# NeLy-EPFL/flygym

Measured on AMD Instinct MI355X. Metric: env-steps/sec (whole node), 4096 flies per GPU, flat terrain, higher is better.
Workload: dtype f32

## Files before the change

flygym_amd/csrc/nmf_capi.hip:

```cpp
#include <algorithm>
#include <cmath>
#include <cstdio>
#include <cstdlib>
#include <cstring>
#include <string>
#include <vector>

#ifndef NMF_DEVMEM_CHECK
#include <hip/hip_runtime.h>

#include "nmf.h"
#include "nmf_batch_ops.hip"
#include "nmf_step.hip"
#include "nmf_sensors.hip"
#include "nmf_eyes.hip"
#include "nmf_camera.hip"
#include "nmf_replay.hip"
#include "nmf_cpg.hip"
#include "nmf_skeleton.h"
#endif

namespace {

thread_local std::string g_err;
// ... 330 lines not shown
      std::vector<int> trn = model->find("act_trn")->i;
      for (int u = 0; u < model->nu; ++u) if ((int)ag->f[(size_t)u * nmf::kActGen] & 1) trn[(size_t)u] = 0;
      upload(b, trn, &d.act_trn);
    }
  }
  UI(geom_body); UI(geom_type); UI(geom_hulladr); UI(geom_hullnum); UI(geom_sensor);
  UF(geom_p0); UF(geom_p1); UF(geom_radius); UF(geom_bsphere); UF(geom_invweight0); UF(hull_vert);
  UF(pair_friction); UF(pair_solref); UF(pair_solimp); UF(pair_margin);
#undef UF
#undef UI
  if (fam.tree_tables()) {
    const HostArray* bp = model->find("body_parent");
    upload(b, bp->i, &d.body_parent);
    upload(b, tree_body, &d.tree_body);
    upload(b, child_start, &d.tree_child_start);
    upload(b, child_count, &d.tree_child_count);
    d.tree_nlevel = (int)lvl_start.size() - 1;
    for (size_t k = 0; k < 18; ++k) d.tree_lvl_start[k] = k < lvl_start.size() ? lvl_start[k] : (int)tree_body.size();
    d.rest_fast = 0; d.rest_pack = nullptr;
    std::vector<int> pack;
    if (fam.hybrid() && !opt.rest_slow && rest_pack_words(model, sk, pack)) { d.rest_fast = 1; upload(b, pack, &d.rest_pack); }
  } else {
    d.body_parent = d.tree_body = d.tree_child_start = d.tree_child_count = nullptr; d.tree_nlevel = 0; d.rest_fast = 0; d.rest_pack = nullptr;
  }
  d.noslip_iter = 0;
  if (const HostArray* os2 = model->find("opt_solver")) { if (os2->i.size() > 1) d.noslip_iter = os2->i[1]; }
  d.max_contacts = nmf::kMaxCon;
  d.solver_flags = opt.solver & 7;
  if (rc != 0) return rc;
  b->dm_dev = (nmf::DevModel*)b->mem.upload(&d, sizeof(nmf::DevModel));
  return b->mem.ok ? 0 : -1;
}

int alloc_state(nmf_batch* b) {
  const nmf_model* model = b->model;
  const size_t n_worlds = (size_t)b->n_worlds;
  nmf::DevState& st = b->st;
  st.n_worlds = b->n_worlds;
  float* stats_sum = nullptr;
  b->handoff_stride = (model->nq + 2 * model->nv + model->nu + 6 + nmf::kActHistWords + 63) / 64 * 64;
  alloc_field(b, NMF_QPOS, model->nq, &st.qpos); alloc_field(b, NMF_QVEL, model->nv, &st.qvel);
  alloc_field(b, NMF_CTRL, model->nu, &st.ctrl); alloc_field(b, NMF_QACC_WARMSTART, model->nv, &st.qacc_ws);
  alloc_field(b, NMF_SEG_XPOS, model->nseg * 3, &st.seg_xpos); alloc_field(b, NMF_SEG_XQUAT, model->nseg * 4, &st.seg_xquat);
  alloc_field(b, NMF_SITE_XPOS, model->nsite * 3, &st.site_xpos); alloc_field(b, NMF_ACTUATOR_FORCE, model->nu, &st.actuator_force);
  alloc_field(b, NMF_SENSORDATA, 96, &st.sensordata); alloc_field(b, NMF_TIME, 1, &st.time);
  alloc_field(b, NMF_STATS, 8, &st.stats); alloc_field(b, NMF_QACC, model->nv, &st.qacc); alloc_field(b, NMF_COST, 1, &st.cost);
  alloc_field(b, NMF_STATS_SUM, 16, &stats_sum);
  alloc_field(b, NMF_CONTACT_GEOM, nmf::kMaxCon, &st.contact_geom); alloc_field(b, NMF_ACT, model->nu, &st.act);
  alloc_dev(b, n_worlds, &b->order_buf); alloc_dev(b, 1, &b->csched_buf);
  alloc_dev(b, n_worlds * (size_t)b->handoff_stride, &b->handoff_buf);
  alloc_dev(b, n_worlds * nmf::kActHistWords, &st.act_hist);
  st.stats_sum = reinterpret_cast<unsigned int*>(stats_sum);
  st.dual_scratch = nullptr;
  with_topo(b->topo, [&](auto tag) { if (nmf::kDualGlob<typename decltype(tag)::type>) alloc_dev(b, n_worlds * nmf::kDualScratchFloats, &st.dual_scratch); });
  st.noslip_buf = nullptr;
  if (b->dm.noslip_iter > 0) alloc_dev(b, n_worlds * nmf::kNoslipFloats, &st.noslip_buf);
  alloc_dev(b, 2, &b->clock_probe_buf); alloc_dev(b, 1, &b->sched_buf);
  st.clock_probe = b->clock_probe_buf;
  st.sched = nullptr;
  st.order = nullptr;
  return b->mem.ok ? 0 : -1;
}

void set_schedule(nmf_batch* b, const Options& opt) {
  b->chunking = opt.sched != 1;
  if (opt.order) b->order_policy = opt.order == 1 ? 0 : opt.order == 2 ? 1 : opt.order == 3 ? 2 : opt.order == 4 ? -1 : 3;
  if (opt.order_every > 0) b->order_every = opt.order_every;
  if (opt.max_chunks > 0) b->max_chunks = std::max(1, std::min(16, opt.max_chunks));
  b->chunk_div = b->dm.terrain_type == 0 ? nmf::family(b->topo).chunk_div : 2.0;
  b->chunk_div_short = true;
  if (opt.chunk_div > 0.0) { b->chunk_div = opt.chunk_div; b->chunk_div_short = false; }
  if (opt.min_chunk_steps > 0) b->min_chunk_steps = opt.min_chunk_steps;
  if (b->dm.act_general) b->chunking = false;
}

int pick_kernel(nmf_batch* b, const Options& opt) {
  const int topo = b->topo, device = b->mem.device;
  int per_cu = nmf::family(topo).per_cu;
  const bool weld = b->dm.weld_active != 0, terrain = b->dm.terrain_type != 0;
  if (weld && terrain) return fail("nmf_batch_create: a tethered world has no terrain");
  const void* fn = step_kernel(topo, weld, terrain);
  if (!fn) return fail("nmf_batch_create: this build of the library has no kernel for the model's skeleton (NMF_TOPO_MASK)");
  int nblk = 0;
  if (hipOccupancyMaxActiveBlocksPerMultiprocessor(&nblk, fn, nmf::kWave, 0) == hipSuccess && nblk > 0) per_cu = nblk;
  b->step_fn = fn;
  const int want = opt.flies_per_cu;
  hipFuncAttributes fa;
  if (want > 0 && want < per_cu && hipFuncGetAttributes(&fa, fn) == hipSuccess) {
    int lds_cu = 0;
    if (hipDeviceGetAttribute(&lds_cu, hipDeviceAttributeMaxSharedMemoryPerMultiprocessor, device) != hipSuccess || lds_cu <= 0) lds_cu = 160 * 1024;
    const int granule = 512;
    int per_wg = (lds_cu / (want + 1) / granule + 1) * granule;
    if (per_wg * want <= lds_cu && per_wg > (int)fa.sharedSizeBytes) {
      b->lds_pad = (unsigned)(per_wg - (int)fa.sharedSizeBytes);
      int nblk2 = 0;
      if (hipOccupancyMaxActiveBlocksPerMultiprocessor(&nblk2, fn, nmf::kWave, b->lds_pad) == hipSuccess && nblk2 > 0) per_cu = std::min(per_cu, nblk2);
      else per_cu = want;
    }
  }
  if (const char* e = dev_env("NMF_LDS_PAD")) b->lds_pad = (unsigned)atoi(e);
  b->per_cu = per_cu;
  hipDeviceProp_t prop;
  b->resident_waves = (hipGetDeviceProperties(&prop, device) == hipSuccess ? prop.multiProcessorCount : 256) * per_cu;
  return 0;
}

}
// ... 807 lines not shown
```

flygym_amd/csrc/nmf_step.hip:

```cpp
#include "nmf_device.h"
#include "nmf_step_lds.h"
#include "nmf_step_diag.h"
#include "nmf_step_kinematics.h"
#include "nmf_step_collision.h"
#include "nmf_step_aba.h"
#include "nmf_step_contact.h"
#include "nmf_dual.h"
#include "nmf_step_noslip.h"
#include "nmf_step_actuation.h"
#include "nmf_step_forward.h"
#include "nmf_step_io.h"
#include "nmf_tree.h"

namespace nmf {

template <class TP> constexpr int waves_per_simd() { return 2; }

template <class TP>
__device__ __forceinline__ void stage_launch_constants(FlyLds<TP>& s, const GModel& m) {
  if constexpr (!TP::kStar) { if (threadIdx.x == 0) { s.rt_nb = m.nb; s.rt_nv = m.nv; } __syncthreads(); }
  if constexpr (TP::kNFact > 1) {
    for (int b = threadIdx.x; b < TP::kTblB && b < m.nb; b += kWave) {
      s.t_body[b] = (unsigned char)m.tree_body[b < m.tree_lvl_start[m.tree_nlevel] ? b : 0];
      s.t_parent[b] = (unsigned char)(b ? m.body_parent[b] : 0);
// ... 31 lines not shown
      }
    }
  }
  if constexpr (kHasIsym<TP>) if (lane == 0) {
    const Frame fr = make_frame(v3(m.plane[0], m.plane[1], m.plane[2]));
    st3(&s.frame9[0], fr.n); st3(&s.frame9[3], fr.t1); st3(&s.frame9[6], fr.t2);
    HotModel& h = s.hot;
    h.dof_axis = m.dof_axis; h.body_pos = m.body_pos; h.body_quat = m.body_quat; h.geom_p0 = m.geom_p0; h.geom_p1 = m.geom_p1;
    h.geom_radius = m.geom_radius; h.geom_bsphere = m.geom_bsphere; h.hull_vert = m.hull_vert; h.pair_margin = m.pair_margin;
    h.geom_body = m.geom_body; h.geom_type = m.geom_type; h.geom_hulladr = m.geom_hulladr; h.geom_hullnum = m.geom_hullnum;
#pragma unroll
    for (int i = 0; i < 4; ++i) h.plane[i] = m.plane[i];
#pragma unroll
    for (int i = 0; i < 5; ++i) h.terrain[i] = m.terrain[i];
    h.hull_skin = m.hull_skin; h.terrain_type = m.terrain_type; h.ng = m.ng; h.sem_max_hull_contacts = m.sem_max_hull_contacts;
    h.terrain_walls = m.sem_terrain_walls;
  }
  if constexpr (kHasIsym<TP>) for (int i = lane; i < 3 * s.nv(); i += kWave) (&s.axis[0][0])[i] = m.dof_axis[i];
}

template <class TP>
__global__ void __launch_bounds__(kWave) nmf_reset_kernel(const DevModel* __restrict__ mp, DevState st, const unsigned char* __restrict__ reset_mask) {
  __shared__ FlyLds<TP> s;
  const GModel& m = *(const GModel*)mp;
  const int lane = threadIdx.x, w = (int)blockIdx.x;
  if (w >= st.n_worlds || (reset_mask && !reset_mask[w])) return;
  stage_launch_constants(s, m);
  for (int i = lane; i < s.nq(); i += kWave) s.qpos[i] = m.key_qpos[i];
  for (int i = lane; i < s.nv(); i += kWave) { s.qvel[i] = 0.f; s.qacc[i] = 0.f; }
  for (int i = lane; i < m.nu; i += kWave) { s.ctrl[i] = m.key_ctrl[i]; st.actuator_force[(size_t)w * m.nu + i] = 0.f; st.act[(size_t)w * m.nu + i] = 0.f; }
  for (int i = lane; i < 96; i += kWave) st.sensordata[(size_t)w * 96 + i] = 0.f;
  if (lane == 0) { s.ncon = 0; s.iters = 0; s.overflow = 0; s.solve_resid = 0.f; }
  WSYNC();
  stage_kinematics(s, m, lane);
  write_poses(s, m, st, w, lane);
  write_outputs(s, m, st, w, lane, 0.f, true);
  if (lane < 16) st.stats_sum[16 * (size_t)w + lane] = 0u;
  if (lane < kActHistWords) st.act_hist[(size_t)w * kActHistWords + lane] = 0u;
  if (lane < kMaxCon) st.contact_geom[(size_t)w * kMaxCon + lane] = -1.f;
}

template <class TP, bool WELD>
__global__ void __launch_bounds__(kWave) __attribute__((amdgpu_waves_per_eu(waves_per_simd<TP>(), waves_per_simd<TP>()))) nmf_step_kernel(const DevModel* __restrict__ mp, DevState st, ReplayArgs rp, int n_steps) {
  __shared__ FlyLds<TP> s;
  const GModel& m = *(const GModel*)mp;
  const unsigned long long probe_c0 = __builtin_amdgcn_s_memtime(), probe_r0 = __builtin_amdgcn_s_memrealtime();
  TRACE_DECL();
  const int lane = threadIdx.x;
  const bool chunked = st.sched_mode == 1;
  unsigned int t_first = 0;
  if (chunked && lane == 0) t_first = atomicAdd(&st.csched->ticket, 1u);
  stage_launch_constants(s, m);
  if constexpr (kDualGlob<TP>) { if (lane == 0) s.dual_glob[0] = st.dual_scratch + (size_t)blockIdx.x * kDualScratchFloats; }
  unsigned int t_next = (unsigned int)__builtin_amdgcn_readfirstlane((int)t_first);
  STAGE_INIT();
  const int n_chunks = chunked ? st.n_chunks : 1;
  const unsigned int epoch = chunked ? (unsigned int)__builtin_amdgcn_readfirstlane((int)st.csched->epoch) : 0u;
  for (;;) {
    int slot = (int)blockIdx.x, chunk = 0, step0 = 0, step1 = n_steps;
    if (chunked) {
      const unsigned int t = t_next;
      if (t >= (unsigned int)st.n_worlds * (unsigned int)n_chunks) {
        if (lane == 0 && atomicAdd(&st.csched->exited, 1u) == gridDim.x - 1u) {
          st.csched->ticket = 0u; st.csched->exited = 0u; st.csched->epoch = epoch + 1u;
        }
        break;
      }
      chunk = (int)(t / (unsigned int)st.n_worlds); slot = (int)(t % (unsigned int)st.n_worlds);
      step0 = st.chunk_start[chunk]; step1 = st.chunk_start[chunk + 1];
    } else if (slot >= st.n_worlds) return;
    const int w = __builtin_amdgcn_readfirstlane(st.order ? st.order[slot] : slot);
    TRACE_SUB(2);
    const unsigned long long t_begin = __builtin_amdgcn_s_memtime();
    if (st.sched && lane == 0) atomicMin(&st.sched->t_first, (unsigned long long)__builtin_amdgcn_s_memrealtime());
    float time;
    unsigned int carry = 0u;
    unsigned int sum_con = 0u, sum_it = 0u, sum_of = 0u;
    unsigned int sum_dual = 0u, sum_kkt = 0u;
    {
      const float* tab = rp.table ? rp.table + (size_t)w * rp.table_steps * rp.n_act : nullptr;
      const int ln = opaque(lane);
      const int my_ctrl = tab && lane < rp.n_act ? rp.act_ids[ln] : -1;
      CtrlPrefetch pf;
      pf.mine = my_ctrl >= 0; pf.next_row = nullptr;
      pf.value = my_ctrl >= 0 ? tab[(size_t)((rp.start + step0) % rp.table_steps) * rp.n_act + lane] : 0.f;
      if (chunk > 0) {
        const unsigned int want = (unsigned int)__builtin_amdgcn_readfirstlane((int)(epoch * 32u + (unsigned int)chunk));
        const unsigned long long* hb = st.handoff + (size_t)w * st.handoff_stride;
        const int nq = s.nq(), nv = s.nv();
        for (;;) {
          bool ok = true;
          for (int i = ln; i < nq; i += kWave) s.qpos[i] = ld_tagged(&hb[i], want, ok);
          for (int i = ln; i < nv; i += kWave) { s.qvel[i] = ld_tagged(&hb[nq + i], want, ok); s.qacc[i] = ld_tagged(&hb[nq + nv + i], want, ok); }
          for (int i = ln; i < m.nu; i += kWave) s.ctrl[i] = ld_tagged(&hb[nq + 2 * nv + i], want, ok);
          carry = lane < 6 ? ld_tagged_u(&hb[nq + 2 * nv + m.nu + ln], want, ok) : 0u;
          if constexpr (kDual<TP>) { const unsigned int hw = lane < hist_words<TP>(m) ? ld_tagged_u(&hb[nq + 2 * nv + m.nu + 6 + ln], want, ok) : 0u; if (lane < kHistLds<TP>) s.act_hist[lane] = hw; }
          if (!__any(!ok)) break;
          __builtin_amdgcn_s_sleep(8);
        }
        time = __uint_as_float((unsigned int)__builtin_amdgcn_readlane((int)carry, 0));
      } else {
        for (int i = ln; i < s.nq(); i += kWave) s.qpos[i] = ld_state(&st.qpos[(size_t)w * s.nq() + i]);
        for (int i = ln; i < s.nv(); i += kWave) {
          s.qvel[i] = ld_state(&st.qvel[(size_t)w * s.nv() + i]);
          s.qacc[i] = ld_state(&st.qacc_ws[(size_t)w * s.nv() + i]);
        }
// ... 77 lines not shown
```

flygym_amd/csrc/nmf_step_aba.h:

```cpp
#pragma once
#include "nmf_device.h"

namespace nmf {

template <class TP> __device__ void tree_sweep_twists(FlyLds<TP>& s, const float* x, float (*T)[row_width_tw<TP>()], const GModel& m, int lane);
template <class TP, class Extra, class Emit>
__device__ __forceinline__ void tree_sweep_project(FlyLds<TP>& s, float (*W)[row_width_tw<TP>()], const GModel& m, int lane, Extra&& extra, Emit&& emit);
template <class TP, bool WELD>
__device__ void tree_aba_solve(FlyLds<TP>& s, int tau_id, int x_id, bool withK, float hdamp, const GModel& m, int lane);
template <class TP> __device__ void tree_sweep_twists_levels(FlyLds<TP>& s, const float* x, float (*T)[row_width_tw<TP>()], const GModel& m, int lane);
template <class TP, class Extra>
__device__ __forceinline__ void tree_gather_levels(FlyLds<TP>& s, float (*W)[row_width_tw<TP>()], const GModel& m, int lane, Extra&& extra);
struct RestNode;
template <class TP, bool FAST, bool UP, class F> __device__ __forceinline__ void rest_levels(FlyLds<TP>& s, int lane, F&& f);
template <class TP, int NUM>
__device__ __forceinline__ void rest_aba_eliminate(FlyLds<TP>& s, const RestNode& nd, const float* tau, bool withK, float hdamp,
                                                   const Frame& fr, const LaneRole& L, const int (&so)[6], const struct InertiaRowMap& IM, const GModel& m);
template <class TP, int NUM, bool HOMOGENEOUS>
__device__ __forceinline__ void rest_aba_expand(FlyLds<TP>& s, const RestNode& nd, float* x, const LaneRole& L);

template <class TP>
__device__ __forceinline__ bool rest_reduced(const FlyLds<TP>& s) {
  if constexpr (TP::kStar) { if constexpr (TP::REST_B > 0) return __builtin_amdgcn_readfirstlane(s.reduced) != 0; }
  return false;
// ... 231 lines not shown
  const float invD = __builtin_amdgcn_rcpf(D);
  const float u = tauj - sp;
  const float k = U * invD;
  const f2 nk = mk2(-k, -k);
  a01 = __builtin_elementwise_fma(nk, mk2(grp8_bcast<0>(U), grp8_bcast<1>(U)), a01);
  a23 = __builtin_elementwise_fma(nk, mk2(grp8_bcast<2>(U), grp8_bcast<3>(U)), a23);
  a45 = __builtin_elementwise_fma(nk, mk2(grp8_bcast<4>(U), grp8_bcast<5>(U)), a45);
  IA[0] = a01.x; IA[1] = a01.y; IA[2] = a23.x; IA[3] = a23.y; IA[4] = a45.x; IA[5] = a45.y;
  pA += k * u;
  UDout = SHADOW0 ? k : mask * k; uDout = u * invD;
  Uraw = U; invDraw = invD;
}
typedef const __attribute__((address_space(3))) float* lds_cptr;
template <class T>
__device__ __forceinline__ lds_cptr lds_pinned(const T* p) {
  lds_cptr q = (lds_cptr)(const void*)p;
  asm("" : "+v"(q));
  return q;
}

template <class TP> __device__ __forceinline__ float (*dual_leg(FlyLds<TP>& s))[8] {
  if constexpr (kDualGlob<TP>) return reinterpret_cast<float(*)[8]>(s.dual_glob[0]);
  else if constexpr (kDualH<TP>) {
    static_assert(!kDualH<TP> || kDualGlob<TP> || 4 * TP::NV >= TP::NLEG * TP::NDL * 8, "leg factors do not fit vA..vD");
    return reinterpret_cast<float(*)[8]>(&s.vA[0]);
  } else {
    static_assert(sizeof(float) * 8 * (TP::NLEG * TP::NDL + 6) <= sizeof(float) * 12 * kMaxCon, "articulated-body factors do not fit c_w + c_m3");
    return reinterpret_cast<float(*)[8]>(&s.c_w[0][0]);
  }
}
template <class TP> __device__ __forceinline__ float (*dual_root(FlyLds<TP>& s))[8] {
  if constexpr (kDualH<TP>) return reinterpret_cast<float(*)[8]>(&s.c_w[0][0]);
  else return dual_leg(s) + TP::NLEG * TP::NDL;
}
template <class TP> __device__ __forceinline__ float* dual_aref(FlyLds<TP>& s) {
  if constexpr (kDualH<TP>) return &s.c_w[0][0] + 48; else return s.vB;
}
template <class TP> __device__ __forceinline__ float (*dual_wrench(FlyLds<TP>& s))[7] {
  if constexpr (kDualH<TP>) {
    static_assert(!kDualH<TP> || 7 * kDualMaxCon<TP> <= TP::NV, "contact wrenches do not fit vC");
    return reinterpret_cast<float(*)[7]>(&s.vC[0]);
  } else return s.c_w;
}
template <class TP> __device__ __forceinline__ float* dual_acc(FlyLds<TP>& s) {
  if constexpr (kDualH<TP>) {
    static_assert(!kDualH<TP> || 96 + TP::NLEG * TP::NDL + 6 <= 7 * kMaxCon, "hinge sums do not fit c_w");
    return &s.c_w[0][0] + 96;
  } else {
    static_assert(TP::NLEG * TP::NDL + 6 <= 3 * TP::NV, "hinge sums do not fit vB..vD");
    return s.vB;
  }
}

template <class TP, bool WELD, bool WITHK_ = true>
__device__ __noinline__ void aba_solve(FlyLds<TP>& s, int tau_id, int x_id, bool withK, float hdamp,
                          const GModel& m, int lane, bool store = false, bool withF = false) {
  if constexpr (!TP::kStar) { tree_aba_solve<TP, WELD>(s, tau_id, x_id, withK, hdamp, m, lane); return; } else {
  withK = WITHK_ && __builtin_amdgcn_readfirstlane((int)withK) != 0;
  store = kDual<TP> && __builtin_amdgcn_readfirstlane((int)store) != 0;
  withF = kDual<TP> && __builtin_amdgcn_readfirstlane((int)withF) != 0;
  const float* tau = s.vec(tau_id);
  float* x = s.vec(x_id);
  Frame fr{};
  if (withK) fr = ld_frame(s, m);
  const bool walls = TP::kTerrain && withK && __builtin_amdgcn_readfirstlane(s.nwall) != 0;
  const LaneRole L = lane_role<TP>(lane);
  const int j0 = TP::LD0 + L.lg * TP::NDL, b0 = TP::LB0 + L.lg * TP::NBL;
  static_assert(sizeof(AbaHandoff<TP>) <= sizeof(float) * TP::NB * 12, "ABA hand-off does not fit T..W");
  AbaHandoff<TP>& H = *reinterpret_cast<AbaHandoff<TP>*>(&s.T[0][0]);
  int so[6];
#pragma unroll
  for (int c = 0; c < 6; c++) {
    if constexpr (kHasIsym<TP>) so[c] = __float_as_int(s.k_tab[L.rr][14 + c]);
    else { const int i = L.rr < c ? L.rr : c, jx = L.rr < c ? c : L.rr; so[c] = i * 6 - i * (i - 1) / 2 + (jx - i); }
  }
  InertiaRowMap IM{};
  if constexpr (!kHasIsym<TP>) IM = inertia_map_unpack(s.k_tab[L.rr]);
  constexpr bool kKeepS = TP::NDL <= 16;
  float Ureg[TP::NDL], ureg[TP::NDL], Sreg[kKeepS ? TP::NDL : 1];
  constexpr bool kShadow0 = row_width_s<TP>() > 6 && row_width_tw<TP>() > 6;
  const int rS = kShadow0 && L.r >= 6 ? 6 : L.rr;
  const lds_cptr Sleg = lds_pinned(&s.S[j0][0]), Sown = lds_pinned(&s.S[j0][rS]);
  constexpr int SW = row_width_s<TP>();
  KLane KL;
  if (withK) {
    const float* q = s.k_tab[L.rr];
#pragma unroll
    for (int i = 0; i < 3; ++i) { KL.dA[i] = q[i]; KL.dB[i] = q[3 + i]; KL.dO[i] = q[6 + i]; }
    KL.ia = __float_as_int(q[9]); KL.ib = __float_as_int(q[10]);
  }
  int cs[TP::NBL + 1], cs_root0 = 0, cs_root1 = 0;
  static_for<TP::NBL + 1>([&](auto I) { constexpr int l = decltype(I)::value; cs[l] = withK || withF ? s.body_cstart[b0 + l] : 0; });
  if (withK || withF) { cs_root0 = s.body_cstart[0]; cs_root1 = s.body_cstart[1]; }
  const bool red = rest_reduced(s);
  SUB_T0();
  if constexpr (TP::REST_B > 0) {
    if (!red) {
      if (m.rest_fast) rest_levels<TP, true, true>(s, lane, [&](const auto& nd) { rest_aba_eliminate<TP, 3>(s, nd, tau, withK, hdamp, fr, L, so, IM, m); });
      else rest_levels<TP, false, true>(s, lane, [&](const auto& nd) { rest_aba_eliminate<TP, 0>(s, nd, tau, withK, hdamp, fr, L, so, IM, m); });
      WSYNC();
    }
  }
  SUB(18);
  float IA[6] = {0.f, 0.f, 0.f, 0.f, 0.f, 0.f};
  float pA = 0.f;
  float n_sj[6], n_sown = 0.f, n_delta = 0.f, n_tau = 0.f, n_row[6];
  auto fetch_hinge = [&](auto DN) {
    constexpr int dn = decltype(DN)::value;
#pragma unroll
    for (int i = 0; i < 6; i++) n_sj[i] = Sleg[dn * SW + i];
    n_sown = Sown[dn * SW];
    n_delta = dof_delta(s, m, j0 + dn, hdamp);
    n_tau = tau[j0 + dn];
    if constexpr (TP::is_last(dn) && kHasIsym<TP>) {
#pragma unroll
      for (int c = 0; c < 6; c++) n_row[c] = s.Isym[b0 + TP::lbody(dn)][so[c]];
    }
  };
  fetch_hinge(std::integral_constant<int, TP::NDL - 1>{});
  static_for<TP::NDL>([&](auto DD) {
    constexpr int d = TP::NDL - 1 - decltype(DD)::value;
    float sj[6], row[6];
#pragma unroll
    for (int i = 0; i < 6; i++) { sj[i] = n_sj[i]; row[i] = n_row[i]; }
    const float sown = n_sown, delta = n_delta, tj = n_tau;
    if constexpr (d > 0) fetch_hinge(std::integral_constant<int, (d > 0 ? d - 1 : 0)>{});
    if constexpr (TP::is_last(d)) {
      const int b = b0 + TP::lbody(d);
      if constexpr (kHasIsym<TP>) {
        if constexpr (kDual<TP>) {
          if (withF) {
#pragma clang loop unroll(disable) vectorize(disable)
            for (int c = cs[TP::lbody(d)]; c < cs[TP::lbody(d) + 1]; ++c) pA -= dual_wrench(s)[c][L.rr];
          }
        }
        if (withK) for (int c = cs[TP::lbody(d)]; c < cs[TP::lbody(d) + 1]; ++c) add_contact_K_row(row, s, c, KL, fr, L.rr, walls);
        add6(IA, row);
      } else {
        add_inertia_row(IA, s, b, IM);
        if constexpr (kDual<TP>) {
          if (withF) {
#pragma clang loop unroll(disable) vectorize(disable)
            for (int c = cs[TP::lbody(d)]; c < cs[TP::lbody(d) + 1]; ++c) pA -= dual_wrench(s)[c][L.rr];
          }
        }
        if (withK) for (int c = cs[TP::lbody(d)]; c < cs[TP::lbody(d) + 1]; ++c) add_contact_K_row(IA, s, c, KL, fr, L.rr, walls);
      }
    }
    const float sr = kShadow0 ? sown : L.mask * sown;
    if constexpr (kKeepS) Sreg[d] = sown;
    float Uraw, invDraw;
    aba_step_scaled<kShadow0>(IA, pA, sj, sr, L.mask, delta, tj, Ureg[d], ureg[d], Uraw, invDraw);
    if constexpr (kDual<TP>) {
      if (store) {
        const float rs = __builtin_sqrtf(invDraw);
        if constexpr (kDualGlob<TP>) ((__attribute__((address_space(1))) float*)s.dual_glob[0])[(L.lg * TP::NDL + d) * 8 + (L.r < 6 ? L.r : 6)] = L.r < 6 ? Uraw * rs : rs;
        else dual_leg(s)[L.lg * TP::NDL + d][L.r < 6 ? L.r : 6] = L.r < 6 ? Uraw * rs : rs;
      }
    }
  });
  constexpr bool kLegSumValu = TP::NLEG <= 8;
  float legs_row[6] = {0.f, 0.f, 0.f, 0.f, 0.f, 0.f}, legs_pA = 0.f;
  if constexpr (kLegSumValu) {
    const float gm = L.grp < TP::NLEG ? 1.f : 0.f;
#pragma unroll
    for (int i = 0; i < 6; i++) legs_row[i] = groups_sum(gm * IA[i]);
    legs_pA = groups_sum(gm * pA);
  } else {
#pragma unroll
    for (int i = 0; i < 6; i++) H.legIA[L.lg][L.rr][i] = IA[i];
    H.legpA[L.lg][L.rr] = pA;
    WSYNC();
  }
  float Ur[6], ur[6];
  float Rm[3][3];
  {
    float row[6] = {0.f, 0.f, 0.f, 0.f, 0.f, 0.f};
    if constexpr (kHasIsym<TP>) {
#pragma unroll
      for (int c = 0; c < 6; c++) row[c] = s.Isym[0][so[c]];
    } else add_inertia_row(row, s, 0, IM);
    if (withK) {
      for (int c = cs_root0; c < cs_root1; ++c) add_contact_K_row(row, s, c, KL, fr, L.rr, walls);
      if constexpr (WELD) static_for<6>([&](auto I) { constexpr int i = decltype(I)::value; row[i] += L.rr == i ? s.weldD[i] : 0.f; });
    }
    pA = 0.f;
    if constexpr (kDual<TP>) {
      if (withF) for (int c = cs_root0; c < cs_root1; ++c) pA -= dual_wrench(s)[c][L.rr];
    }
    if constexpr (kLegSumValu) { add6(row, legs_row); pA += legs_pA; }
    else {
#pragma unroll
      for (int k = 0; k < TP::NLEG; ++k) {
        add6(row, H.legIA[k][L.rr]);
        pA += H.legpA[k][L.rr];
      }
    }
    if constexpr (TP::REST_B > 0) {
      if (red) {
#pragma unroll
        for (int i = 0; i < 6; i++) row[i] += s.restA[so[i]];
      } else {
        if (!withK && hdamp == 0.f && lane < 21) {
          float a = 0.f;
          for (int k = (int)s.t_cstart[0]; k < (int)s.t_cstart[0] + (int)s.t_ccount[0]; ++k) a += s.slot_at(k - 1)[lane];
          s.restA[lane] = a;
        }
        for (int k = (int)s.t_cstart[0]; k < (int)s.t_cstart[0] + (int)s.t_ccount[0]; ++k) {
          const float* sl = s.slot_at(k - 1);
          { float v[6];
#pragma unroll
            for (int i = 0; i < 6; i++) v[i] = sl[so[i]];
            add6(row, v); }
          pA += sl[21 + L.rr];
        }
      }
    }
#pragma unroll
    for (int i = 0; i < 6; i++) IA[i] = row[i];
#pragma unroll
    for (int k = 0; k < 3; k++)
#pragma unroll
      for (int c = 0; c < 3; c++) Rm[c][k] = s.S[3 + k][c];
    float tw[6];
    const float t3 = tau[3], t4 = tau[4], t5 = tau[5];
#pragma unroll
    for (int c = 0; c < 3; c++) { tw[c] = Rm[c][0] * t3 + Rm[c][1] * t4 + Rm[c][2] * t5; tw[3 + c] = tau[c]; }
    static_for<6>([&](auto DD) {
      constexpr int i = decltype(DD)::value;
      constexpr int e = i < 3 ? 2 - i : 8 - i;
      const float U = IA[e];
      const float b0 = grp8_bcast<0>(U), b1 = grp8_bcast<1>(U), b2 = grp8_bcast<2>(U), b3 = grp8_bcast<3>(U),
                  b4 = grp8_bcast<4>(U), b5 = grp8_bcast<5>(U);
      const float D = e == 0 ? b0 : e == 1 ? b1 : e == 2 ? b2 : e == 3 ? b3 : e == 4 ? b4 : b5;
      const float sp = grp8_bcast<e>(pA);
      const float invD = __builtin_amdgcn_rcpf(D);
      const float u = tw[e] - sp;
      const float k = U * invD;
      { const float bb[6] = {b0, b1, b2, b3, b4, b5}; fma6(IA, -k, bb); }
      pA += k * u;
      Ur[e] = kShadow0 ? k : L.mask * k; ur[e] = u * invD;
      if constexpr (kDual<TP>) {
        if (store) {
          const float rs = __builtin_sqrtf(invD);
          dual_root(s)[i][L.r < 6 ? L.r : 6] = L.r < 6 ? U * rs : rs;
        }
      }
    });
  }
  float a = 0.f;
  {
    float xw[6];
    static_for<6>([&](auto DD) {
      constexpr int i = decltype(DD)::value;
      constexpr int e = i < 3 ? 3 + i : i - 3;
      const float xe = ur[e] - grp8_sum(Ur[e] * a);
      xw[e] = xe;
      a = (kShadow0 ? L.r : L.rr) == e ? a + xe : a;
    });
#pragma unroll
    for (int k = 0; k < 3; k++) {
      x[k] = xw[3 + k];
      x[3 + k] = Rm[0][k] * xw[0] + Rm[1][k] * xw[1] + Rm[2][k] * xw[2];
    }
  }
  s.T[0][rS] = a;
  static_for<TP::NDL>([&](auto DD) {
    constexpr int d = decltype(DD)::value;
    const int j = j0 + d;
    const float xj = ureg[d] - grp8_sum(Ureg[d] * a);
    x[j] = xj;
    if constexpr (kKeepS) a += xj * Sreg[d]; else a += xj * Sown[d * SW];
    if constexpr (TP::is_last(d)) s.T[b0 + TP::lbody(d)][rS] = a;
  });
  WSYNC();
  SUB(19);
  if constexpr (TP::REST_B > 0) {
    if (!red) {
      if (m.rest_fast) rest_levels<TP, true, false>(s, lane, [&](const auto& nd) { rest_aba_expand<TP, 3, false>(s, nd, x, L); });
      else rest_levels<TP, false, false>(s, lane, [&](const auto& nd) { rest_aba_expand<TP, 0, false>(s, nd, x, L); });
    }
  }
  SUB(20);
  }
}

}
```

flygym_amd/csrc/nmf_step_forward.h:

```cpp
#pragma once
#include "nmf_device.h"

namespace nmf {

template <class TP> __device__ void tree_velocity_bias(FlyLds<TP>& s, const GModel& m, int lane);

template <class TP, bool WELD>
__device__ bool physics_forward(FlyLds<TP>& s, const GModel& m, int lane, const DevState& st, int w, bool last, float* rec, CtrlPrefetch& pf STAGE_ARG) {
  if constexpr (TP::kStar) { if constexpr (TP::REST_B > 0 || TP::kTerrain) lane = opaque(lane); }
  const Frame fr = make_frame(v3(m.plane[0], m.plane[1], m.plane[2]));
  if constexpr (TP::kStar) { if constexpr (TP::REST_B > 0) { if (lane == 0) s.reduced = 0; } }
  stage_kinematics(s, m, lane);
  STAGE(1);
  stage_inertia(s, m, lane);
  STAGE(2);
  stage_collision<TP, TP::kTerrain>(s, m, lane);
  if (pf.next_row && pf.mine) pf.value = G(pf.next_row)[lane];
  if (last) write_poses(s, m, st, w, lane);
  STAGE(3);
  const int ncon = s.ncon;
  const bool walls = TP::kTerrain && __builtin_amdgcn_readfirstlane(s.nwall) != 0;

  ContactRegs c;
  auto rows = [&](SV t, float* out) {
// ... 473 lines not shown
  for (int dest = 0; dest < 2; ++dest) {
    float* out = dest == 0 ? (last ? &st.sensordata[(size_t)w * 96] : nullptr) : (rec ? rec + 2 * st.ring_nj + st.ring_nact : nullptr);
    if (!out) continue;
    const int ol = opaque(lane);
    for (int i = ol; i < 96; i += kWave) out[i] = 0.f;
    WSYNC();
    if (m.nsensor && lane < 6 && smask) {
      float wsum = 0.f; V3 pc = v3(0, 0, 0), pm = v3(0, 0, 0), F = v3(0, 0, 0), Tq = v3(0, 0, 0); int cnt = 0;
      Frame f1 = fr;
      for (unsigned long long mk = smask; mk; mk &= mk - 1ull) {
        const int cc = __ffsll((long long)mk) - 1;
        V3 f = ld3(&s.c_w[cc][3]);
        const Frame cf = walls ? contact_frame(info_fid(s.c_info[cc]), fr) : fr;
        if (cnt == 0) f1 = cf;
        float fn = dot(f, cf.n);
        V3 p = ld3(s.c_r[cc]);
        wsum += fn; pc = pc + fn * p; pm = pm + p; cnt++;
      }
      pc = wsum > 0.f ? (1.0f / wsum) * pc : (1.0f / (float)cnt) * pm;
      for (unsigned long long mk = smask; mk; mk &= mk - 1ull) {
        const int cc = __ffsll((long long)mk) - 1;
        V3 f = ld3(&s.c_w[cc][3]);
        F = F + f;
        Tq = Tq + cross(ld3(s.c_r[cc]) - pc, f);
      }
      float* o16 = out + 16 * ol;
      V3 o = ld3(s.xpos()[0]);
      if (m.sem_sensor_contact_frame) {
        F = v3(dot(f1.n, F), dot(f1.t1, F), dot(f1.t2, F));
        Tq = v3(dot(f1.n, Tq), dot(f1.t1, Tq), dot(f1.t2, Tq));
      }
      o16[0] = (float)cnt; st3(o16 + 1, F); st3(o16 + 4, Tq); st3(o16 + 7, pc + o); st3(o16 + 10, f1.n); st3(o16 + 13, f1.t1);
    }
  }
  WSYNC();
  STAGE(17);
  return solved;
}

template <class TP, bool WELD>
__device__ void physics_integrate(FlyLds<TP>& s, const GModel& m, int lane, bool wrenches STAGE_ARG) {
  if constexpr (TP::kStar) { if constexpr (TP::REST_B > 0 || TP::kTerrain) lane = opaque(lane); }
  const Frame fr = make_frame(v3(m.plane[0], m.plane[1], m.plane[2]));
  const float h = m.timestep;
  wrenches = __builtin_amdgcn_readfirstlane((int)wrenches) != 0;
  if (wrenches) {
    if constexpr (kDualH<TP>) {
      if (lane < s.ncon) {
#pragma unroll
        for (int i = 0; i < 6; ++i) dual_wrench(s)[lane][i] = s.c_w[lane][i];
      }
      WSYNC();
    }
    aba_solve<TP, WELD, !kDual<TP>>(s, V_QFRC_SMOOTH, V_B, false, h, m, lane, false, true);
  }
  else {
    for (int j = lane; j < s.nv(); j += kWave) s.vA[j] = s.qfrc_smooth[j] + s.vD[j];
    WSYNC();
    aba_solve<TP, WELD, !kDual<TP>>(s, V_A, V_B, false, h, m, lane);
  }
  const Q4 q0 = ldq(&s.qpos[3]);
  float v0 = 0.f;
  if constexpr (TP::kStar) {
    if constexpr (TP::NV > kWave && TP::NV <= 2 * kWave) {
      const int jb = lane + kWave;
      const bool two = jb < TP::NV;
      const float va = s.qvel[lane] + h * s.vB[lane];
      const float pa = lane >= 6 ? s.qpos[lane + 1] : 0.f;
      float vb2 = 0.f, pb = 0.f;
      if (two) { vb2 = s.qvel[jb] + h * s.vB[jb]; pb = s.qpos[jb + 1]; }
      s.qvel[lane] = va;
      if (lane >= 6) s.qpos[lane + 1] = pa + h * va;
      if (two) { s.qvel[jb] = vb2; s.qpos[jb + 1] = pb + h * vb2; }
      v0 = va;
    }
  }
  if (!(TP::kStar && TP::NV > kWave && TP::NV <= 2 * kWave)) {
    for (int j = lane; j < s.nv(); j += kWave) {
      const float v = s.qvel[j] + h * s.vB[j];
      s.qvel[j] = v;
      if (j >= 6) s.qpos[j + 1] += h * v;
      if (j < kWave) v0 = v;
    }
  }
  {
    const V3 w = v3(readlane_f(v0, 3), readlane_f(v0, 4), readlane_f(v0, 5));
    if (lane < 3) s.qpos[lane] += h * v0;
    const float wn = sqrtf(dot(w, w));
    Q4 q = q0;
    if (wn > kMinVal) {
      float sn, cs;
      sincos_bounded(0.5f * h * wn, &sn, &cs);
      V3 ax = (sn / wn) * w;
      q = qmul(q, Q4{cs, ax.x, ax.y, ax.z});
    }
    q = qnorm(q);
    if (lane == 0) stq(&s.qpos[3], q);
  }
  WSYNC();
}

}
```

flygym_amd/csrc/nmf_step_lds.h:

```cpp
#pragma once
#include "nmf_device.h"

namespace nmf {

#define WSYNC() do { __builtin_amdgcn_fence(__ATOMIC_SEQ_CST, "wavefront"); __builtin_amdgcn_wave_barrier(); } while (0)
constexpr float kNoiseFactor = 8.f;
enum : unsigned int {
  kExitDual = 1u << 8,
  kExitKkt = 1u << 9,
  kExitTie = 1u << 10,
  kExitStall = 1u << 11,
  kExitCost = 1u << 12,
  kExitMaxIter = 1u << 13,
  kExitPrimal = 1u << 14,
  kExitFallback = 1u << 15,
  kExitBigPivots = 1u << 16,
  kExitNoNoslip = 1u << 17,
  kExitFree = 1u << 18,
};
constexpr int kExitKinds = 12;
constexpr int kDualRegPivots = 47;
constexpr float kDualResidMax = 1e-3f;
constexpr int kDualExitFrom = 5;

#define NMF_TREE_TABLES                                                                                                  \
  unsigned char t_body[TP::kTblB], t_parent[TP::kTblB], t_dofadr[TP::kTblB], t_dofnum[TP::kTblB], t_cstart[TP::kTblB],    \
      t_ccount[TP::kTblB], t_dofbody[TP::kTblV];                                                                          \
  unsigned char t_lvl[18], t_nlevel;

template <class TP, bool STAR = TP::kStar, bool REST = (TP::kNFact > 1)>
struct TreeLds {};
template <class TP>
struct TreeLds<TP, false, true> {
  float fact[TP::kNFact][8];
  float slot[TP::kNSlot][27];
  int rt_nb, rt_nv;
  NMF_TREE_TABLES
};
template <class TP>
struct TreeLds<TP, true, true> {
  float fact[TP::kNFact][8];
  int reduced;
  float restA[21];
  unsigned int t_pack[kRestLevels][8][2];
  NMF_TREE_TABLES
};

template <class TP> constexpr bool has_cm3() { if constexpr (TP::kStar) return TP::REST_B == 0; else return false; }
template <class TP> inline constexpr bool kHasCm3 = has_cm3<TP>();
template <class TP> inline constexpr bool kHasIsym = has_cm3<TP>();

constexpr bool rows_conflict_free(int rows_per_leg, int width, int nleg) {
  const int ng = nleg < 4 ? nleg : 4;
  for (int a = 0; a < ng; ++a)
    for (int b = a + 1; b < ng; ++b) {
      const int d = (((b - a) * rows_per_leg * width) % 32 + 32) % 32;
      if (d < 6 || d > 26) return false;
    }
  return true;
}
constexpr int conflict_free_width(int rows_per_leg, int nleg) {
  for (int w = 6; w <= 9; ++w) if (rows_conflict_free(rows_per_leg, w, nleg)) return w;
  return 6;
}
template <class TP> constexpr int row_width_s() { if constexpr (TP::kStar) return TP::REST_B == 0 ? conflict_free_width(TP::NDL, TP::NLEG) : 6; else return 6; }
template <class TP> constexpr int row_width_tw() { if constexpr (TP::kStar) return TP::REST_B == 0 ? conflict_free_width(TP::NBL, TP::NLEG) : 6; else return 6; }
template <class TP> constexpr bool dual_hybrid() {
  if constexpr (TP::kStar) return TP::REST_B > 0; else return false;
}
template <class TP> constexpr bool dual_global() {
  if constexpr (TP::kStar) return TP::REST_B > 0 && 4 * TP::NV < TP::NLEG * TP::NDL * 8; else return false;
}
template <class TP> inline constexpr bool kDualS = has_cm3<TP>();
template <class TP> inline constexpr bool kDualH = dual_hybrid<TP>();
template <class TP> inline constexpr bool kDual = kDualS<TP> || kDualH<TP>;
template <class TP> inline constexpr bool kDualGlob = kDualH<TP> && dual_global<TP>();
constexpr int kDualScratchFloats = 8 * 6 * 24;
constexpr int dual_g_floats(int ncon) { return 9 * ncon * (ncon + 1) / 2; }
template <class TP> constexpr int dual_max_con() {
  if constexpr (kDualH<TP>) {
    int n = 0;
    while (n < 16 && dual_g_floats(n + 1) <= 2 * TP::NB * 6) ++n;
    return n;
  } else return 16;
}
template <class TP> inline constexpr int kDualMaxCon = dual_max_con<TP>();
template <class TP> inline constexpr int kHistLds = kDualS<TP> ? kActHistWords : kDualH<TP> ? 5 : 0;
template <class TP, class M> __device__ __forceinline__ int hist_words(const M& m) {
  if constexpr (kDualS<TP>) return (m.ng + 1) / 2; else return kHistLds<TP>;
}
template <class TP> constexpr int dual_pad_floats() {
  if constexpr (kDualS<TP>) {
    constexpr int need = dual_g_floats(kDualMaxCon<TP>);
    constexpr int have = TP::NB * 11 + 2 * TP::NB * (TP::REST_B == 0 ? conflict_free_width(TP::NBL, TP::NLEG) : 6);
    return need > have ? need - have : 0;
  } else return 0;
}

struct HotModel {
  const float *dof_axis, *body_pos, *body_quat, *geom_p0, *geom_p1, *geom_radius, *geom_bsphere, *hull_vert, *pair_margin;
  const int *geom_body, *geom_type, *geom_hulladr, *geom_hullnum;
  float plane[4], terrain[5], hull_skin;
  int terrain_type, ng, sem_max_hull_contacts, terrain_walls;
};
template <class TP> struct FlyLds;
template <class TP> struct AbaHandoff;
template <class T> using gptr = const __attribute__((address_space(1))) T*;
template <class T> __device__ __forceinline__ gptr<T> G(const T* p) { return (gptr<T>)p; }
__device__ __forceinline__ V3 ld3(gptr<float> p) { return V3{p[0], p[1], p[2]}; }
__device__ __forceinline__ Q4 ldq(gptr<float> p) { return Q4{p[0], p[1], p[2], p[3]}; }

template <class TP>
struct __align__(16) FlyLds : TreeLds<TP> {
  __device__ __forceinline__ int nv() const { if constexpr (TP::kStar) return TP::NV; else return this->rt_nv; }
  __device__ __forceinline__ int nb() const { if constexpr (TP::kStar) return TP::NB; else return this->rt_nb; }
  __device__ __forceinline__ int nq() const { return nv() + 1; }
  float qpos[TP::NQ + 3];
  float qvel[TP::NV], qacc[TP::NV];
  float xmat_root[9];
  float qacc_smooth[TP::NV], qfrc_smooth[TP::NV];
  float vA[TP::NV], vB[TP::NV], vC[TP::NV], vD[TP::NV];
  float ctrl[TP::kCtrl];
  float S[TP::NV][row_width_s<TP>()];
  float Isym[kHasIsym<TP> ? TP::NB : 1][kHasIsym<TP> ? 21 : 1];
  alignas(kDualS<TP> ? 16 : 4) float Ib[TP::NB][kHasCm3<TP> ? 11 : 10];
  static_assert(6 * TP::NV >= 9 * (TP::NB - 1), "rotation matrices do not fit the solver vectors");
  static_assert(7 * kMaxCon >= 3 * (TP::NB - 1), "body positions do not fit the contact wrenches");
  __device__ __forceinline__ float (*xmat())[9] { return reinterpret_cast<float(*)[9]>(&xmat_root[0]); }
  __device__ __forceinline__ const float (*xmat() const)[9] { return reinterpret_cast<const float(*)[9]>(&xmat_root[0]); }
  __device__ __forceinline__ float (*xpos())[3] { return reinterpret_cast<float(*)[3]>(&xpos_root[0]); }
  __device__ __forceinline__ const float (*xpos() const)[3] { return reinterpret_cast<const float(*)[3]>(&xpos_root[0]); }
  float T[TP::NB][row_width_tw<TP>()], W[TP::NB][row_width_tw<TP>()];
  float dual_pad[dual_pad_floats<TP>()];
  float arm[TP::NV], damp[kHasCm3<TP> ? TP::NV : 1];
  float dlt[kHasCm3<TP> ? TP::NV : 1];
  float c_r[kMaxCon][3], c_D[kMaxCon], c_mu[kMaxCon];
  int c_info[kMaxCon];
  alignas(kDualS<TP> ? 16 : 4) float xpos_pad_[kDualS<TP> ? 1 : 0];
  float xpos_root[3];
  float c_w[kMaxCon][7];
  float c_m3[kHasCm3<TP> ? kMaxCon : 1][kHasCm3<TP> ? 5 : 1];
  float k_tab[6][kHasIsym<TP> ? 20 : 14];
  float frame9[kHasIsym<TP> ? 9 : 1];
  std::conditional_t<kHasIsym<TP>, HotModel, char> hot;
  float axis[kHasIsym<TP> ? TP::NV : 1][3];
  float weldD[6], weld_w[6];
  using cstart_t = std::conditional_t<kHasIsym<TP>, int, unsigned char>;
  cstart_t body_cstart[(TP::NB + 1 + 3) / 4 * 4];
  __device__ __forceinline__ float* slot_at(int k) {
    if constexpr (TP::kStar) {
      constexpr int kInCw = 7 * kMaxCon / 27;
      static_assert(TP::REST_B == 0 || (TP::REST_B - kInCw) * 27 * sizeof(float) + sizeof(AbaHandoff<TP>) <= sizeof(float) * TP::NB * 2 * row_width_tw<TP>(),
                    "hand-off slots of the rest do not fit T..W");
      return k < kInCw ? &c_w[0][0] + 27 * k : &T[0][0] + sizeof(AbaHandoff<TP>) / sizeof(float) + 27 * (k - kInCw);
    } else return this->slot[k];
  }
  unsigned int act_hist[kHistLds<TP>];
  float* dual_glob[kDualGlob<TP> ? 1 : 0];
  int ncon, overflow;
  int iters;
  float solve_resid;
  int nwall;
  __device__ __forceinline__ float* vec(int id) {
    switch (id) {
      case 0: return qacc;
      case 1: return qacc_smooth;
      case 2: return qfrc_smooth;
      case 3: return vA;
      case 4: return vB;
      case 5: return vC;
      default: return vD;
    }
  }
};
template <class TP> __device__ __forceinline__ HotModel hot_model(const FlyLds<TP>& s, const GModel& m) {
  if constexpr (kHasIsym<TP>) return s.hot;
  else {
// ... 95 lines not shown
```

Before: 62.83 million.

## Reuse Euler ABA factorization via global scratch instead of refactoring each solve

During the first ABA solve (with K), a second inertia-only factorization is computed alongside and its per-dof k and 1/D factors are written to a per-block global scratch buffer. Later Euler-step solves that previously reran a full ABA factorization now call a new aba_solve_stored. It loads those factors and performs only the forward and back substitutions. This trades redundant factorization arithmetic for extra work and global-memory stores in the first solve, plus a scratch allocation and more register pressure.

```diff
diff --git a/flygym_amd/csrc/nmf_capi.hip b/flygym_amd/csrc/nmf_capi.hip
--- a/flygym_amd/csrc/nmf_capi.hip
+++ b/flygym_amd/csrc/nmf_capi.hip
@@ -406,7 +406,11 @@
   alloc_dev(b, n_worlds * nmf::kActHistWords, &st.act_hist);
   st.stats_sum = reinterpret_cast<unsigned int*>(stats_sum);
   st.dual_scratch = nullptr;
-  with_topo(b->topo, [&](auto tag) { if (nmf::kDualGlob<typename decltype(tag)::type>) alloc_dev(b, n_worlds * nmf::kDualScratchFloats, &st.dual_scratch); });
+  with_topo(b->topo, [&](auto tag) {
+    using TP = typename decltype(tag)::type;
+    if (nmf::kDualGlob<TP>) alloc_dev(b, n_worlds * nmf::kDualScratchFloats, &st.dual_scratch);
+    else if (nmf::kEulerFused<TP>) alloc_dev(b, n_worlds * (size_t)nmf::euler_scratch_floats<TP>(), &st.dual_scratch);
+  });
   st.noslip_buf = nullptr;
   if (b->dm.noslip_iter > 0) alloc_dev(b, n_worlds * nmf::kNoslipFloats, &st.noslip_buf);
   alloc_dev(b, 2, &b->clock_probe_buf); alloc_dev(b, 1, &b->sched_buf);
diff --git a/flygym_amd/csrc/nmf_step.hip b/flygym_amd/csrc/nmf_step.hip
--- a/flygym_amd/csrc/nmf_step.hip
+++ b/flygym_amd/csrc/nmf_step.hip
@@ -107,6 +107,12 @@
   if (chunked && lane == 0) t_first = atomicAdd(&st.csched->ticket, 1u);
   stage_launch_constants(s, m);
   if constexpr (kDualGlob<TP>) { if (lane == 0) s.dual_glob[0] = st.dual_scratch + (size_t)blockIdx.x * kDualScratchFloats; }
+  if constexpr (kEulerFused<TP>) {
+    if (lane == 0) {
+      const unsigned long long p = (unsigned long long)(st.dual_scratch + (size_t)blockIdx.x * euler_scratch_floats<TP>());
+      s.euler_fac[0] = (unsigned int)p; s.euler_fac[1] = (unsigned int)(p >> 32);
+    }
+  }
   unsigned int t_next = (unsigned int)__builtin_amdgcn_readfirstlane((int)t_first);
   STAGE_INIT();
   const int n_chunks = chunked ? st.n_chunks : 1;
diff --git a/flygym_amd/csrc/nmf_step_aba.h b/flygym_amd/csrc/nmf_step_aba.h
--- a/flygym_amd/csrc/nmf_step_aba.h
+++ b/flygym_amd/csrc/nmf_step_aba.h
@@ -307,6 +307,26 @@
   }
 }
 
+typedef __attribute__((address_space(1))) float* euler_fac_ptr;
+template <class TP> __device__ __forceinline__ euler_fac_ptr euler_fac_base(FlyLds<TP>& s) {
+  if constexpr (kEulerFused<TP>) {
+    const unsigned int lo = (unsigned int)__builtin_amdgcn_readfirstlane((int)s.euler_fac[0]);
+    const unsigned int hi = (unsigned int)__builtin_amdgcn_readfirstlane((int)s.euler_fac[1]);
+    return (euler_fac_ptr)((unsigned long long)hi << 32 | lo);
+  } else return nullptr;
+}
+template <int e>
+__device__ __forceinline__ void aba_root_factor(float (&IA)[6], float& kout, float& invDout) {
+  const float U = IA[e];
+  const float b0 = grp8_bcast<0>(U), b1 = grp8_bcast<1>(U), b2 = grp8_bcast<2>(U), b3 = grp8_bcast<3>(U),
+              b4 = grp8_bcast<4>(U), b5 = grp8_bcast<5>(U);
+  const float D = e == 0 ? b0 : e == 1 ? b1 : e == 2 ? b2 : e == 3 ? b3 : e == 4 ? b4 : b5;
+  const float invD = __builtin_amdgcn_rcpf(D);
+  const float k = U * invD;
+  { const float bb[6] = {b0, b1, b2, b3, b4, b5}; fma6(IA, -k, bb); }
+  kout = k; invDout = invD;
+}
+
 template <class TP, bool WELD, bool WITHK_ = true>
 __device__ __noinline__ void aba_solve(FlyLds<TP>& s, int tau_id, int x_id, bool withK, float hdamp,
                           const GModel& m, int lane, bool store = false, bool withF = false) {
@@ -314,6 +334,8 @@
   withK = WITHK_ && __builtin_amdgcn_readfirstlane((int)withK) != 0;
   store = kDual<TP> && __builtin_amdgcn_readfirstlane((int)store) != 0;
   withF = kDual<TP> && __builtin_amdgcn_readfirstlane((int)withF) != 0;
+  constexpr bool kFuse = kEulerFused<TP> && !WITHK_;
+  if constexpr (kFuse) { withF = false; hdamp = 0.f; }
   const float* tau = s.vec(tau_id);
   float* x = s.vec(x_id);
   Frame fr{};
@@ -337,6 +359,8 @@
   const int rS = kShadow0 && L.r >= 6 ? 6 : L.rr;
   const lds_cptr Sleg = lds_pinned(&s.S[j0][0]), Sown = lds_pinned(&s.S[j0][rS]);
   constexpr int SW = row_width_s<TP>();
+  euler_fac_ptr fac = nullptr, fac_root = nullptr;
+  if constexpr (kFuse) { fac = euler_fac_base(s) + (L.lg * 8 + (L.r < 6 ? L.r : 6)); fac_root = euler_fac_base(s) + (TP::NLEG * TP::NDL * 8 + (L.r < 6 ? L.r : 6)); }
   KLane KL;
   if (withK) {
     const float* q = s.k_tab[L.rr];
@@ -358,14 +382,16 @@
   }
   SUB(18);
   float IA[6] = {0.f, 0.f, 0.f, 0.f, 0.f, 0.f};
+  float IAe[6] = {0.f, 0.f, 0.f, 0.f, 0.f, 0.f};
   float pA = 0.f;
-  float n_sj[6], n_sown = 0.f, n_delta = 0.f, n_tau = 0.f, n_row[6];
+  float n_sj[6], n_sown = 0.f, n_delta = 0.f, n_delta_e = 0.f, n_tau = 0.f, n_row[6];
   auto fetch_hinge = [&](auto DN) {
     constexpr int dn = decltype(DN)::value;
 #pragma unroll
     for (int i = 0; i < 6; i++) n_sj[i] = Sleg[dn * SW + i];
     n_sown = Sown[dn * SW];
     n_delta = dof_delta(s, m, j0 + dn, hdamp);
+    if constexpr (kFuse) n_delta_e = s.dlt[j0 + dn];
     n_tau = tau[j0 + dn];
     if constexpr (TP::is_last(dn) && kHasIsym<TP>) {
 #pragma unroll
@@ -378,7 +404,7 @@
     float sj[6], row[6];
 #pragma unroll
     for (int i = 0; i < 6; i++) { sj[i] = n_sj[i]; row[i] = n_row[i]; }
-    const float sown = n_sown, delta = n_delta, tj = n_tau;
+    const float sown = n_sown, delta = n_delta, delta_e = n_delta_e, tj = n_tau;
     if constexpr (d > 0) fetch_hinge(std::integral_constant<int, (d > 0 ? d - 1 : 0)>{});
     if constexpr (TP::is_last(d)) {
       const int b = b0 + TP::lbody(d);
@@ -391,6 +417,7 @@
         }
         if (withK) for (int c = cs[TP::lbody(d)]; c < cs[TP::lbody(d) + 1]; ++c) add_contact_K_row(row, s, c, KL, fr, L.rr, walls);
         add6(IA, row);
+        if constexpr (kFuse) add6(IAe, row);
       } else {
         add_inertia_row(IA, s, b, IM);
         if constexpr (kDual<TP>) {
@@ -406,6 +433,11 @@
     if constexpr (kKeepS) Sreg[d] = sown;
     float Uraw, invDraw;
     aba_step_scaled<kShadow0>(IA, pA, sj, sr, L.mask, delta, tj, Ureg[d], ureg[d], Uraw, invDraw);
+    if constexpr (kFuse) {
+      float pe = 0.f, UDe, uDe, Ue, invDe;
+      aba_step_scaled<kShadow0>(IAe, pe, sj, sr, L.mask, delta_e, 0.f, UDe, uDe, Ue, invDe);
+      fac[(TP::NDL - 1 - d) * TP::NLEG * 8] = L.r < 6 ? Ue * invDe : invDe;
+    }
     if constexpr (kDual<TP>) {
       if (store) {
         const float rs = __builtin_sqrtf(invDraw);
@@ -416,10 +448,16 @@
   });
   constexpr bool kLegSumValu = TP::NLEG <= 8;
   float legs_row[6] = {0.f, 0.f, 0.f, 0.f, 0.f, 0.f}, legs_pA = 0.f;
+  float legs_row_e[6] = {0.f, 0.f, 0.f, 0.f, 0.f, 0.f};
+  static_assert(!kFuse || kLegSumValu, "the fused factor sweep sums the legs on the VALU");
   if constexpr (kLegSumValu) {
     const float gm = L.grp < TP::NLEG ? 1.f : 0.f;
 #pragma unroll
     for (int i = 0; i < 6; i++) legs_row[i] = groups_sum(gm * IA[i]);
+    if constexpr (kFuse) {
+#pragma unroll
+      for (int i = 0; i < 6; i++) legs_row_e[i] = groups_sum(gm * IAe[i]);
+    }
     legs_pA = groups_sum(gm * pA);
   } else {
 #pragma unroll
@@ -442,6 +480,11 @@
     pA = 0.f;
     if constexpr (kDual<TP>) {
       if (withF) for (int c = cs_root0; c < cs_root1; ++c) pA -= dual_wrench(s)[c][L.rr];
+    }
+    if constexpr (kFuse) {
+#pragma unroll
+      for (int i = 0; i < 6; i++) IAe[i] = row[i];
+      add6(IAe, legs_row_e);
     }
     if constexpr (kLegSumValu) { add6(row, legs_row); pA += legs_pA; }
     else {
@@ -495,6 +538,11 @@
       { const float bb[6] = {b0, b1, b2, b3, b4, b5}; fma6(IA, -k, bb); }
       pA += k * u;
       Ur[e] = kShadow0 ? k : L.mask * k; ur[e] = u * invD;
+      if constexpr (kFuse) {
+        float ke, invDe;
+        aba_root_factor<e>(IAe, ke, invDe);
+        fac_root[i * 8] = L.r < 6 ? ke : invDe;
+      }
       if constexpr (kDual<TP>) {
         if (store) {
           const float rs = __builtin_sqrtf(invD);
@@ -540,4 +588,103 @@
   }
 }
 
-}
+template <class TP>
+__device__ __noinline__ void aba_solve_stored(FlyLds<TP>& s, int tau_id, int x_id, const GModel& m, int lane, bool withF) {
+  static_assert(kEulerFused<TP> && TP::NLEG <= 8 && TP::NDL <= 16, "leg-chain kernels");
+  withF = __builtin_amdgcn_readfirstlane((int)withF) != 0;
+  SUB_T0();
+  SUB(18);
+  const LaneRole L = lane_role<TP>(lane);
+  constexpr int NE = TP::NDL + 6;
+  float Fk[NE], Fd[NE];
+  {
+    const euler_fac_ptr fk = euler_fac_base(s) + (L.lg * 8 + L.rr), fd = euler_fac_base(s) + (L.lg * 8 + 6);
+    const euler_fac_ptr rk = euler_fac_base(s) + (TP::NLEG * TP::NDL * 8 + L.rr), rd = euler_fac_base(s) + (TP::NLEG * TP::NDL * 8 + 6);
+#pragma unroll
+    for (int e = 0; e < TP::NDL; ++e) { Fk[e] = fk[e * TP::NLEG * 8]; Fd[e] = fd[e * TP::NLEG * 8]; }
+#pragma unroll
+    for (int i = 0; i < 6; ++i) { Fk[TP::NDL + i] = rk[i * 8]; Fd[TP::NDL + i] = rd[i * 8]; }
+  }
+  const float* tau = s.vec(tau_id);
+  float* x = s.vec(x_id);
+  const int j0 = TP::LD0 + L.lg * TP::NDL, b0 = TP::LB0 + L.lg * TP::NBL;
+  constexpr bool kShadow0 = row_width_s<TP>() > 6 && row_width_tw<TP>() > 6;
+  const int rS = kShadow0 && L.r >= 6 ? 6 : L.rr;
+  const lds_cptr Sown = lds_pinned(&s.S[j0][rS]);
+  constexpr int SW = row_width_s<TP>();
+  int cs[TP::NBL + 1], cs_root0 = 0, cs_root1 = 0;
+  static_for<TP::NBL + 1>([&](auto I) { constexpr int l = decltype(I)::value; cs[l] = withF ? s.body_cstart[b0 + l] : 0; });
+  if (withF) { cs_root0 = s.body_cstart[0]; cs_root1 = s.body_cstart[1]; }
+  float Ureg[TP::NDL], ureg[TP::NDL], sown[TP::NDL], tj[TP::NDL];
+#pragma unroll
+  for (int d = 0; d < TP::NDL; ++d) { sown[d] = Sown[d * SW]; tj[d] = tau[j0 + d]; }
+  float pA = 0.f;
+  static_for<TP::NDL>([&](auto DD) {
+    constexpr int d = TP::NDL - 1 - decltype(DD)::value;
+    if constexpr (TP::is_last(d)) {
+      if (withF) {
+#pragma clang loop unroll(disable) vectorize(disable)
+        for (int c = cs[TP::lbody(d)]; c < cs[TP::lbody(d) + 1]; ++c) pA -= dual_wrench(s)[c][L.rr];
+      }
+    }
+    const float sr = kShadow0 ? sown[d] : L.mask * sown[d];
+    const float k = Fk[TP::NDL - 1 - d], invD = Fd[TP::NDL - 1 - d];
+    const float sp = grp8_sum(sr * pA);
+    const float u = tj[d] - sp;
+    pA += k * u;
+    Ureg[d] = kShadow0 ? k : L.mask * k; ureg[d] = u * invD;
+  });
+  const float gm = L.grp < TP::NLEG ? 1.f : 0.f;
+  const float legs_pA = groups_sum(gm * pA);
+  float Ur[6], ur[6], Rm[3][3];
+  {
+    pA = 0.f;
+    if (withF) for (int c = cs_root0; c < cs_root1; ++c) pA -= dual_wrench(s)[c][L.rr];
+    pA += legs_pA;
+#pragma unroll
+    for (int k = 0; k < 3; k++)
+#pragma unroll
+      for (int c = 0; c < 3; c++) Rm[c][k] = s.S[3 + k][c];
+    float tw[6];
+    const float t3 = tau[3], t4 = tau[4], t5 = tau[5];
+#pragma unroll
+    for (int c = 0; c < 3; c++) { tw[c] = Rm[c][0] * t3 + Rm[c][1] * t4 + Rm[c][2] * t5; tw[3 + c] = tau[c]; }
+    static_for<6>([&](auto DD) {
+      constexpr int i = decltype(DD)::value;
+      constexpr int e = i < 3 ? 2 - i : 8 - i;
+      const float k = Fk[TP::NDL + i], invD = Fd[TP::NDL + i];
+      const float sp = grp8_bcast<e>(pA);
+      const float u = tw[e] - sp;
+      pA += k * u;
+      Ur[e] = kShadow0 ? k : L.mask * k; ur[e] = u * invD;
+    });
+  }
+  float a = 0.f;
+  {
+    float xw[6];
+    static_for<6>([&](auto DD) {
+      constexpr int i = decltype(DD)::value;
+      constexpr int e = i < 3 ? 3 + i : i - 3;
+      const float xe = ur[e] - grp8_sum(Ur[e] * a);
+      xw[e] = xe;
+      a = (kShadow0 ? L.r : L.rr) == e ? a + xe : a;
+    });
+#pragma unroll
+    for (int k = 0; k < 3; k++) {
+      x[k] = xw[3 + k];
+      x[3 + k] = Rm[0][k] * xw[0] + Rm[1][k] * xw[1] + Rm[2][k] * xw[2];
+    }
+  }
+  s.T[0][rS] = a;
+  static_for<TP::NDL>([&](auto DD) {
+    constexpr int d = decltype(DD)::value;
+    const float xj = ureg[d] - grp8_sum(Ureg[d] * a);
+    x[j0 + d] = xj;
+    a += xj * sown[d];
+    if constexpr (TP::is_last(d)) s.T[b0 + TP::lbody(d)][rS] = a;
+  });
+  WSYNC();
+  SUB(19);
+}
+
+}
diff --git a/flygym_amd/csrc/nmf_step_forward.h b/flygym_amd/csrc/nmf_step_forward.h
--- a/flygym_amd/csrc/nmf_step_forward.h
+++ b/flygym_amd/csrc/nmf_step_forward.h
@@ -549,12 +549,14 @@
       }
       WSYNC();
     }
-    aba_solve<TP, WELD, !kDual<TP>>(s, V_QFRC_SMOOTH, V_B, false, h, m, lane, false, true);
+    if constexpr (kEulerFused<TP>) aba_solve_stored<TP>(s, V_QFRC_SMOOTH, V_B, m, lane, true);
+    else aba_solve<TP, WELD, !kDual<TP>>(s, V_QFRC_SMOOTH, V_B, false, h, m, lane, false, true);
   }
   else {
     for (int j = lane; j < s.nv(); j += kWave) s.vA[j] = s.qfrc_smooth[j] + s.vD[j];
     WSYNC();
-    aba_solve<TP, WELD, !kDual<TP>>(s, V_A, V_B, false, h, m, lane);
+    if constexpr (kEulerFused<TP>) aba_solve_stored<TP>(s, V_A, V_B, m, lane, false);
+    else aba_solve<TP, WELD, !kDual<TP>>(s, V_A, V_B, false, h, m, lane);
   }
   const Q4 q0 = ldq(&s.qpos[3]);
   float v0 = 0.f;
diff --git a/flygym_amd/csrc/nmf_step_lds.h b/flygym_amd/csrc/nmf_step_lds.h
--- a/flygym_amd/csrc/nmf_step_lds.h
+++ b/flygym_amd/csrc/nmf_step_lds.h
@@ -76,6 +76,15 @@
 template <class TP> inline constexpr bool kDual = kDualS<TP> || kDualH<TP>;
 template <class TP> inline constexpr bool kDualGlob = kDualH<TP> && dual_global<TP>();
 constexpr int kDualScratchFloats = 8 * 6 * 24;
+template <class TP> constexpr bool euler_fused() {
+#ifdef NMF_EULER_REFACTOR
+  return false;
+#else
+  return has_cm3<TP>();
+#endif
+}
+template <class TP> inline constexpr bool kEulerFused = euler_fused<TP>();
+template <class TP> constexpr int euler_scratch_floats() { if constexpr (has_cm3<TP>()) return 8 * (TP::NLEG * TP::NDL + 6); else return 0; }
 constexpr int dual_g_floats(int ncon) { return 9 * ncon * (ncon + 1) / 2; }
 template <class TP> constexpr int dual_max_con() {
   if constexpr (kDualH<TP>) {
@@ -123,6 +132,7 @@
   float ctrl[TP::kCtrl];
   float S[TP::NV][row_width_s<TP>()];
   float Isym[kHasIsym<TP> ? TP::NB : 1][kHasIsym<TP> ? 21 : 1];
+  unsigned int euler_fac[kEulerFused<TP> ? 2 : 0];
   alignas(kDualS<TP> ? 16 : 4) float Ib[TP::NB][kHasCm3<TP> ? 11 : 10];
   static_assert(6 * TP::NV >= 9 * (TP::NB - 1), "rotation matrices do not fit the solver vectors");
   static_assert(7 * kMaxCon >= 3 * (TP::NB - 1), "body positions do not fit the contact wrenches");
```

After: 64.26 million (median of 6 runs). 1.02x the previous value.
